# lbroseus/TALC

Measured on AMD Instinct MI355X. Metric: corrected long-read bases/sec (whole node); k-mer-probe HBM GB/s, higher is better.
Workload: dtype u8

## Files before the change

talc_amd/csrc/talc_capi_correct.inc:

```

static uint32_t next_launch_stamp() {
  static std::atomic<uint32_t> launches{0};
  return 0x01000000u + (launches.fetch_add(1) & 0xFFFFFFu);
}
static void ensure_edge_boxes(talc_ctx* c, Stage& st) {
  const uint64_t gap = (uint64_t)c->p.max_border_length + 256;
  const uint32_t seqCap = (uint32_t)align_up((uint64_t)(2.2 * (double)gap) + 4ull * c->p.k + 64, 16);
  const uint64_t need = (uint64_t)st.n_slots * edge_box_bytes(seqCap) + (uint64_t)st.n_slots * 4;
  if (c->sw.edgeTasks == 0 || c->p.max_start_anchors < 2 || c->p.max_start_anchors > EDGE_BOX_ANCHORS ||
      seqCap > (1u << 16) || need > (1ull << 30)) {
    st.boxes.reset(); st.boxes_bytes = 0;
    return;
  }
  if (need > st.boxes_bytes || seqCap != st.box_seq_cap) {
    st.boxes.reset(); st.boxes_bytes = 0;
    if (st.boxes.alloc(need) != hipSuccess) { (void)hipGetLastError(); return; }
    st.boxes_bytes = need; st.box_seq_cap = seqCap;
  }
}

static int ensure_stage(talc_ctx* c, Stage& st, uint32_t maxLen, uint32_t scale, uint32_t n_work) {
  const SearchCaps caps = make_caps(maxLen, c->p.k, scale, scale == 1 ? c->sw.seqArena : 0, scale == 1 && c->sw.tinyCaps);
  hipDeviceProp_t prop;
  HIPCHK(hipGetDeviceProperties(&prop, c->device));
// ... 114 lines not shown
  HIPCHK(hipEventRecord(c->ev[3], s));
  return TALC_OK;
}

static int order_queue(talc_ctx* c, talc_batch* b) {
  if (!b->n_reads) return TALC_OK;
  hipStream_t s = c->stream;
  uint32_t* const hist = c->d_hist.get();
  HIPCHK(hipMemsetAsync(hist, 0, kOrderBuckets * sizeof(uint32_t), s));
  const unsigned nb = (b->n_reads + 255) / 256;
  hipLaunchKernelGGL(k_order_scale, dim3(1), dim3(64), 0, s, batch_stats(c));
  hipLaunchKernelGGL(k_order_hist, dim3(nb), dim3(256), 0, s, b->d_state.get(), b->n_reads, hist, batch_stats(c));
  hipLaunchKernelGGL(k_order_scan, dim3(1), dim3(kOrderBuckets), 0, s, hist);
  hipLaunchKernelGGL(k_order_scatter, dim3(nb), dim3(256), 0, s, b->d_state.get(), b->n_reads, hist, b->d_order.get(), batch_stats(c));
  HIPCHK(hipGetLastError());
  return TALC_OK;
}

static int launch_search(talc_ctx* c, talc_batch* b, const Stage& st, const uint32_t* d_work, uint32_t n_work, const TraceBuf& tb,
                         uint32_t traceRead, bool edgeTasks) {
  hipStream_t s = c->stream;
  HIPCHK(hipMemsetAsync(c->d_queue.get(), 0, kQueueWords * sizeof(uint32_t), s));
  EdgeTaskArgs ea = {};
  ea.test = c->sw.edgeLane ? 0u : kTestNoEdgeLane;
  if (edgeTasks && st.boxes) {
    ea.boxes = st.boxes.get();
    ea.avail = (uint32_t*)(st.boxes.get() + (uint64_t)st.n_slots * edge_box_bytes(st.box_seq_cap));
    ea.seqCap = st.box_seq_cap;
    ea.minWeak = c->sw.edgeTaskMin; ea.heavy = c->sw.edgeTaskHeavy; ea.heavyRounds = c->sw.edgeTaskRounds;
    ea.lingerMod = c->sw.edgeLingerMod; ea.test |= c->sw.edgeRedo ? kTestEdgeRedo : 0u;
    ea.autoSwitch = c->sw.edgeTasks > 0 ? nullptr : batch_stats(c) + kStatBranching;
    HIPCHK(hipMemsetAsync(ea.avail, 0, (uint64_t)st.n_slots * 4, s));
  }
  hipLaunchKernelGGL(k_search, dim3(st.n_slots), dim3(64), 0, s, c->dp, c->view, st.caps, b->d_codes.get(), b->d_offsets.get(),
                     b->d_koff.get(), b->d_cov.get(), b->d_covw.get(), b->d_state.get(), b->d_regions.get(), b->d_regoff.get(), b->d_headcov.get(),
                     c->map ? b->d_regions.get() : nullptr, c->map ? b->d_mapedge.get() : nullptr, b->d_out.get(), b->d_outoff.get(), d_work,
                     n_work, c->d_queue.get(), st.scratch.get(), c->d_counters.get(), tb, traceRead, next_launch_stamp(), ea);
  HIPCHK(hipGetLastError());
  return TALC_OK;
}

static int search_first_pass(talc_ctx* c, talc_batch* b, const TraceBuf& tb, uint32_t traceRead) {
  hipStream_t s = c->stream;
  int rc;
  HIPCHK(hipMemsetAsync(c->d_counters.get(), 0, kCounterWords * sizeof(uint64_t), s));
  HIPCHK(hipMemsetAsync(c->d_counters.get() + kCntFirstStart, 0xFF, sizeof(uint64_t), s));
  HIPCHK(hipMemsetAsync(c->d_counters.get() + kCntQueueDry, 0xFF, sizeof(uint64_t), s));
// ... 483 lines not shown
```

talc_amd/csrc/talc_kernels_search.h:

```cpp
#pragma once
#include "talc_common.h"
#include "talc_kernels_probe.h"
#include "talc_pure.h"
#include "talc_wave.h"

namespace talc {

#define TCAP 288
#define NBUF (2 * TCAP)
#ifndef LDS_DP_CAP
#define LDS_DP_CAP 320
#endif
#ifndef HOT
#define HOT 8
#endif
#ifndef AIMS_LDS
#define AIMS_LDS 16
#endif

enum : uint32_t {
  OVF_ANCHORS = 1, OVF_FULLPATHS = 2, OVF_FULLPOOL = 4, OVF_TRAILS = 8, OVF_SEQ = 16, OVF_OUT = 32, OVF_WEAKPOOL = 64,
  OVF_REGIONS = 128, OVF_DP = 256
};

// ... 10 lines not shown
  uint32_t pfHead, pfTail, pfGapSum, pfFork, pfSolid, pfTicks;
  uint32_t pfGapSq, pfGapMax, pfShortReg, pfSteps;
  uint32_t pfBridges, pfBridgeMax;
  uint32_t pfEdgeTicks, pfAnchors, pfAnchorMax, pfStart;
#endif
};

__host__ __device__ inline uint64_t out_capacity_for(uint64_t L) { return 4 * L + 1024; }

struct FullMeta { uint32_t off, len; int32_t lanc, ranc; double dist; };

static const uint32_t kQueueWords = 768, kQueueFinished = 256, kQueueOpen = 512;

static const uint32_t kOrderBuckets = 1024, kBatchStatsOff = kOrderBuckets, kBatchStatsWords = 256, kHistWords = kBatchStatsOff + kBatchStatsWords;
static const uint32_t kStatGapScale = 128, kStatBranching = 129;

static const uint32_t kCntSteps = 0, kCntCells = 1, kCntProf0 = 2, kCntQueueDry = 124, kCntBusy = 125, kCntFirstStart = 126, kCntLastEnd = 127;
static const uint32_t kCntWaveLog = 128, kCntMaxWaves = 8192, kCounterWords = kCntWaveLog + 2 * kCntMaxWaves;

enum { PF_PROBE = 0, PF_CHILD, PF_AIMS, PF_CYCLE, PF_FFWD, PF_SCOREBR, PF_GARDEN, PF_EVALFULL, PF_XDROP, PF_EXTNW,
       PF_EDGEMISC, PF_ANCHORS, PF_ASSEMBLE, PF_STEPB, PF_STEPE, PF_SRCHB, PF_SRCHE, PF_PROLOG, PF_INITTR, PF_TOTAL, PF_NCALLS, PF_NSTEPS,
       PF_FFLOAD, PF_FFREC, PF_FFFLUSH, PF_FFENTRY, PF_NRECS, PF_RD0, PF_RD1, PF_RD2, PF_RD3, PF_RD4, PF_RD5, PF_RDMAX,
       PF_XSTAGE, PF_XLEV, PF_XSEL, PF_REFB, PF_RESULT, PF_CYQ, PF_CYX, PF_CYHIT, PF_CYFILL,
       PF_SB11, PF_SB12, PF_SB21, PF_SB10, PF_SBOTHER, PF_SEGEN, PF_XCALLS, PF_XNLEV, PF_FSFORK, PF_FSDEAD, PF_FSFILT, PF_FSLIM, PF_FK1, PF_FK2, PF_FKBAIL, PF_FORK, PF_ANCCALLS, PF_ANCITER, PF_TPUB, PF_TOWN, PF_TSTOLEN, PF_TWAIT, PF_TRUN, PF_EA0, PF_EA1, PF_EA2, PF_EA3, PF_EA4, PF_EASUM3, PF_EASUM4, PF_RANCH, PF_RANCHMAX, PF_RBR, PF_RBRMAX, PF_EDGELANE, PF_N };
#define TALC_PF_NAMES {"probe", "child", "aims", "cycle", "ffwd", "scorebr", "garden", "evalfull", "xdrop", "extnw", "edgemisc", \
                       "anchors", "assemble", "stepb*", "stepe*", "srchb*", "srche*", "prolog", "inittr", "total", "#ffcalls", "#ffsteps", \
                       "ff.load", "ff.record", "ff.flush", "ff.entry", "#ffrecords", "#reads<0.25ms", "#reads<1ms", "#reads<4ms", \
                       "#reads<16ms", "#reads<64ms", "#reads>=64ms", "maxread(10ns)", "x.stage", "x.levels", "x.select", "b.ref", "b.result", \
                       "#cyc.query", "#cyc.exact", "#cyc.found", "cyc.fill%sum", \
                       "#stepb 1->1", "#stepb 1->2", "#stepb 2->1", "#stepb 1->0", "#stepb other", "#stepe generic", "#xdrop calls", "#xdrop levels", \
                       "#ffstop fork", "#ffstop deadend", "#ffstop filter", "#ffstop limit/other", "#forkstep 1 child", "#forkstep fork+deadend", "#forkstep bailed", "forkstep", "#anchor lists", "#anchor level tests", \
                       "#edges published", "#anchors by owner", "#anchors by others", "t.owner waits", "t.run by others", \
                       "#edge anchors<1ms", "#edge anchors<4ms", "#edge anchors<16ms", "#edge anchors<64ms", "#edge anchors>=64ms", "ticks anchors 16-64ms", "ticks anchors>=64ms", "(per read) anchors", "(per read) longest anchor", "(per read) bridge attempts", "(per read) longest bridge attempt", "edgelane*"}
static_assert(kCntProf0 + PF_N <= kCntQueueDry, "the profile categories run into the utilisation counters");

struct SearchLimits {
  uint32_t seqCap;
  uint32_t seqArena;
  uint32_t refCap;
  uint32_t edgeCap;
  uint32_t anchCap;
  uint32_t fullCap;
  uint32_t fullPool;
  uint32_t dpCap;
  uint32_t regCap;
  uint32_t weakPool;
};
struct SearchCaps : SearchLimits {
  uint64_t slotBytes;
  uint64_t o_setA, o_setB, o_seqPool, o_ref, o_ancL, o_ancR, o_ancPos, o_fullMeta, o_fullPoolB, o_edgeLong,
      o_edgeShort, o_edgeTmp, o_dp, o_gard, o_regS, o_regE, o_wOff, o_wLen, o_weak, o_wideBloom, o_rowPool, o_regH, o_trace;
};

#ifndef ROW_ARENA_INTS
#define ROW_ARENA_INTS (448 * 1024)
#endif
// ... 466 lines not shown
  s.kmer = (uint64_t*)(meta + TrailSetLayout::kmer); s.nmask = (uint64_t*)(meta + TrailSetLayout::nmask);
  s.dist = (double*)(meta + TrailSetLayout::dist); s.cnt = (uint32_t*)(meta + TrailSetLayout::cnt);
  s.score = (int32_t*)(meta + TrailSetLayout::score); s.fail = (uint32_t*)(meta + TrailSetLayout::fail);
  s.lanc = (int32_t*)(meta + TrailSetLayout::lanc); s.ranc = (int32_t*)(meta + TrailSetLayout::ranc);
  s.buf = (uint32_t*)(meta + TrailSetLayout::buf);
  return s;
}

struct TrailRec { uint64_t kmer, nmask; double dist; uint32_t cnt; int32_t score; uint32_t fail; int32_t lanc, ranc; uint32_t buf; };

#define LSYNC() do { __builtin_amdgcn_fence(__ATOMIC_ACQ_REL, "wavefront"); __builtin_amdgcn_wave_barrier(); } while (0)

__shared__ TrailRec g_hot[2 * HOT];
__shared__ uint64_t g_aimK[AIMS_LDS], g_aimN[AIMS_LDS];
__shared__ uint32_t g_aimPos[AIMS_LDS];
#define BLOOM_WORDS 128
__shared__ unsigned long long g_bloom[BLOOM_WORDS];
__shared__ __attribute__((aligned(16))) int g_dp[3 * LDS_DP_CAP];

struct EdgeCand {
  bool have; double score; double dist; double idscore; uint32_t len; uint32_t lanc, ranc;
};

enum : uint32_t { kTestEdgeRedo = 1u, kTestNoEdgeLane = 2u };

struct Wv {
  DevParams P; TableView T; SearchLimits C;
  const uint8_t* read; uint32_t L, n; const uint2* cov; double lambda;
  TrailSet G[2];
  int ia;
  uint8_t* seqPool;
  uint32_t nBuf;
  unsigned long long freeMask[NBUF / 64];
  uint8_t *ref, *fullPool, *edgeLong, *edgeShort, *edgeTmp, *weak;
  AnchorRec *ancL, *ancR; uint32_t* ancPos;
  FullMeta* fullMeta;
  int *dpG;
  double* gScores; double* gDists; ValIdx* gVal; Rank4* gRank; uint32_t* gKept;
  uint32_t *regS, *regE, *wOff, *wLen;
  int location, dirRight;
  uint32_t Ls, Le, Rs, Re;
  uint32_t weakLen;
  bool complexRegion;
  bool ffPopped;
  int nAncL, nAncR;
  uint32_t refLen;
  int nFull; uint32_t fullUsed;
  EdgeCand best2[2];
  int nEdges;
  unsigned long long cells, steps;
  uint32_t overflow;
  const TraceBuf* tracep;
  bool tracing, traceSteps;
  unsigned long long* wideBloom;
  int* rowPool;
  uint32_t searchNo;
  uint32_t rowStride, rowAvail;
  uint32_t wideMask;
  uint32_t launchStamp;
  const CovWord* covw;
  uint32_t* regH;
  uint32_t LH, RH;
  const uint32_t* headCov;
  uint8_t* refBuf;
  uint8_t* boxes; uint32_t* avail; uint32_t* qwords;
  uint32_t* mapRegions; uint32_t* mapEdge;
  uint32_t boxBytes, boxSeqCap, nSlots, mySlot, nWork, taskMinWeak;
// ... 1630 lines not shown

  flush();
  g_bloom[l] = ((unsigned long long)(uint32_t)bwHi << 32) | (uint32_t)bwLo;
  g_bloom[l + 64] = ((unsigned long long)(uint32_t)bxHi << 32) | (uint32_t)bxLo;
  stepCounter_ = sc0 + (uint32_t)done;
  PROF_COUNT(PF_NCALLS, 1); PROF_COUNT(PF_NSTEPS, done);
  if (done) {
    X.steps += (unsigned long long)done;
    if (l == 0) {
      TrailRec r = r0;
      r.kmer = kmer; r.cnt = cnt; r.dist = dist;
      tr_put(X.ia, 0, r);
    }
  }
  LSYNC();
  return done;
}

template <int P>
TALC_D uint32_t dpp_row_shr(uint32_t v, uint32_t old) {
  return (uint32_t)__builtin_amdgcn_update_dpp((int)old, (int)v, 0x110 + P, 0xF, 0xF, false);
}

struct WalkLanes { uint32_t laneOff, laneShift, laneSingle; int lj; };
struct WalkTip { uint64_t kmer, key; uint32_t hh, cnt; uint32_t ePre; bool havePre; int done, flushed; };
template <bool dirRight, bool WIDEF, class Also>
TALC_D int walk_record(const WalkLanes& WL, WalkTip& W, int room, const uint32_t TALC_AS1* wtab, uint64_t cap, uint32_t K, gu8 seq, int len0,
                       uint32_t* recN, int nAims, uint32_t wideMask, unsigned long long* wideBloom, int& nOK, int& aimIdx, Also also) {
  PROF_DECL;
  const int l = lane_id();
  const uint64_t kmask = (1ULL << (2 * K)) - 1, m1 = (1ULL << (2 * (K - 1))) - 1;
  const uint32_t laneOff = WL.laneOff, laneShift = WL.laneShift, laneSingle = WL.laneSingle;
  const int lj = WL.lj;
  uint64_t& kmer = W.kmer; uint64_t& key = W.key; uint32_t& hh = W.hh; uint32_t& cnt = W.cnt; uint32_t& ePre = W.ePre; bool& havePre = W.havePre;
  int& done = W.done; const int flushed = W.flushed;
  nOK = 0; aimIdx = -1;
    PROF_BEGIN();
    uint64_t slot = ((uint64_t)hh * (uint64_t)(uint32_t)cap) >> 32;
    uint32_t e = havePre ? ePre : wtab[slot * 8 + laneOff];
    havePre = false;
    bool found = true;
    while (true) {
      const uint64_t bk = ((uint64_t)(uint32_t)lane_get((int)e, TALC_WALK_LEVELS + 1) << 32) | (uint32_t)lane_get((int)e, TALC_WALK_LEVELS);
      if (bk == key) break;
      if (bk == kEmptyKey) { found = false; break; }
      if (++slot == cap) slot = 0;
      e = wtab[slot * 8 + laneOff];
    }
    PROF_END(PF_FFLOAD);
    PROF_COUNT(PF_NRECS, 1);
    if (!found) return 0;
    PROF_BEGIN();
    const uint32_t lev = (e >> laneShift) & 0xFFFFu, top = lev & kWalkTopNone;
#ifdef TALC_PROF
    {
      const unsigned long long pm = ballot64((l < TALC_WALK_LEVELS) && (lev & kWalkSingle) != 0u);
      const int j0 = __builtin_ctzll(~pm);
      if (j0 < TALC_WALK_LEVELS && j0 < room) {
        const uint32_t t0 = (uint32_t)lane_get((int)top, j0);
        if (l == 0) g_prof[(t0 >= X.P.MIN_COUNT) ? PF_FSFORK : PF_FSDEAD] += 1;
      }
    }
#endif
    const unsigned long long passMask = ballot64((lev & laneSingle) != 0u);
    nOK = min(__builtin_ctzll(~passMask), room);
    if (nOK == 0) return 0;
    const uint32_t which = (l < TALC_WALK_LEVELS) ? (lev >> kWalkBaseShift) : 0u;
    uint32_t pre = which << (dirRight ? 2 * (TALC_WALK_LEVELS - 1 - lj) : 2 * lj);
    pre |= dpp_row_shr<1>(pre, 0u);
    pre |= dpp_row_shr<2>(pre, 0u);
    pre |= dpp_row_shr<4>(pre, 0u);
    pre |= dpp_row_shr<8>(pre, 0u);
    uint64_t km;
    if (dirRight) km = ((kmer << (2 * (lj + 1))) | (uint64_t)(pre >> (2 * (TALC_WALK_LEVELS - 1 - lj)))) & kmask;
    else km = ((uint64_t)pre << (2 * (K - 1 - (uint32_t)lj))) | (kmer >> (2 * (lj + 1)));
    const uint64_t key2 = dirRight ? (km & m1) : (km >> 2);
    const uint32_t hv = (uint32_t)(table_hash(key2) >> 32);
    {
      const uint64_t slotN = ((uint64_t)(uint32_t)lane_get((int)hv, TALC_WALK_LEVELS - 1) * (uint64_t)(uint32_t)cap) >> 32;
      ePre = wtab[slotN * 8 + laneOff];
    }
    bool dup = dpp_row_shr<1>(hv, ~hv) == hv;
    dup |= dpp_row_shr<2>(hv, ~hv) == hv;
    dup |= dpp_row_shr<3>(hv, ~hv) == hv;
    dup |= dpp_row_shr<4>(hv, ~hv) == hv;
    dup |= dpp_row_shr<5>(hv, ~hv) == hv;
    dup |= dpp_row_shr<6>(hv, ~hv) == hv;
    dup |= dpp_row_shr<7>(hv, ~hv) == hv;
    dup |= dpp_row_shr<8>(hv, ~hv) == hv;
    dup |= dpp_row_shr<9>(hv, ~hv) == hv;
    dup |= dpp_row_shr<10>(hv, ~hv) == hv;
    dup |= dpp_row_shr<11>(hv, ~hv) == hv;
    static_assert(TALC_WALK_LEVELS == 12, "the lane roles above are written for 12 levels (+ 2 key lanes) in a 16-lane row");
    const int bwi = (int)(hv >> 25);
    const unsigned long long bm = (1ull << ((hv >> 19) & 63u)) | (1ull << ((hv >> 13) & 63u));
    bool seen = (g_bloom[bwi] & bm) == bm;
    unsigned long long* const wideW = WIDEF ? wideBloom + wide_word(hv, wideMask) : nullptr;
    const unsigned long long bmW = WIDEF ? wide_bits(hv) : 0ull;
    if (WIDEF) {
      const bool ask = seen && (l < TALC_WALK_LEVELS);
      if (ballot64(ask) != 0ull) { const unsigned long long bvW = ask ? wide_load(wideW) : 0ull; seen = ask && ((bvW & bmW) == bmW); }
    }
    const unsigned long long hitMask = ballot64(seen || dup) | (1ull << TALC_WALK_LEVELS);
    const int hitLevel = __builtin_ctzll(hitMask);
    aimIdx = -1;
    if (nAims > 0 && nAims <= AIMS_LDS && hitLevel < nOK) {
      const uint64_t kmH = ((uint64_t)(uint32_t)lane_get((int)(uint32_t)(km >> 32), hitLevel) << 32) | (uint32_t)lane_get((int)(uint32_t)km, hitLevel);
      const unsigned long long am = ballot64((l < nAims) && (g_aimK[l < AIMS_LDS ? l : 0] == kmH) && (g_aimN[l < AIMS_LDS ? l : 0] == 0ull));
      if (am != 0ull) aimIdx = (int)__builtin_ctzll(am);
    }
    if (hitLevel < nOK && aimIdx < 0) PROF_COUNT(PF_FSFILT, 1);
    nOK = min(nOK, hitLevel);
    const int nTake = nOK + (aimIdx >= 0 ? 1 : 0);
    if (nTake == 0) return 0;
    if (l < nTake) {
      atomicOr(&g_bloom[bwi], bm);
      if (WIDEF) wide_or(wideW, bmW);
      recN[done - flushed + l] = top;
      seq[len0 + done + l] = (uint8_t)which;
      also(len0 + done + l, which);
    }
    const int last = nTake - 1;
    kmer = ((uint64_t)(uint32_t)lane_get((int)(uint32_t)(km >> 32), last) << 32) | (uint32_t)lane_get((int)(uint32_t)km, last);
    key = dirRight ? (kmer & m1) : (kmer >> 2);
    hh = (uint32_t)lane_get((int)hv, last);
    havePre = (last == TALC_WALK_LEVELS - 1);
    cnt = (uint32_t)lane_get((int)top, last);
    done += nTake;
    LSYNC();
    PROF_END(PF_FFREC);
  return nTake;
}
TALC_D void walk_flush(WalkTip& W, uint32_t* recN, uint32_t& cFlush, double& dist) {
  const int l = lane_id();
  int& done = W.done; int& flushed = W.flushed;
  const int n = done - flushed;
  if (n <= 0) return;
  PROF_DECL; PROF_BEGIN();
  const uint32_t cn = (l < n) ? recN[l] : 1u;
  const uint32_t cprev = (l == 0) ? cFlush : ((l < n) ? recN[l - 1] : 1u);
  const double term = fabs((double)cprev - (double)cn) / sqrt((double)cprev);
  double* recT = (double*)(g_dp + 64);
  recT[l] = term;
  LSYNC();
#pragma unroll 8
  for (int j = 0; j < n; ++j) dist = dist + recT[j];
  cFlush = (uint32_t)lane_get((int)cn, n - 1);
  flushed = done;
  LSYNC();
  PROF_END(PF_FFFLUSH);
}

template <bool dirRight, bool WIDEF>
TALC_D int fast_forward_walk(int len_, uint32_t& stepCounter_, uint32_t PATH_MAXLENGTH_, bool edge_) {
  PROF_DECL2;
  PROF_BEGIN2();
  const DevParams& P = X.P;
  const int l = lane_id();
  const bool edge = uni((int)edge_) != 0;
  if (uni((int)(X.traceSteps)) != 0) return 0;
  const TrailRec r0 = tr_get(X.ia, 0);
  if (uni64(r0.nmask) != 0ull) return 0;
  const uint32_t K = (uint32_t)uni((int)P.K), CHECK = (uint32_t)uni((int)P.CHECK_INTERVAL);
  const uint32_t seqCap = (uint32_t)uni((int)X.C.seqCap), PMAX = (uint32_t)uni((int)PATH_MAXLENGTH_);
  const uint64_t cap = uni64(X.T.capacity);
  const uint32_t TALC_AS1* wtab = (const uint32_t TALC_AS1*)uni_ptr(dirRight ? X.T.walkRight : X.T.walkLeft);
  const uint32_t wideMask = WIDEF ? (uint32_t)uni((int)X.wideMask) : 0u;
  unsigned long long* const wideBloom = WIDEF ? (unsigned long long*)uni_ptr(X.wideBloom) : nullptr;
  const uint64_t m1 = (1ULL << (2 * (K - 1))) - 1;
  WalkTip W;
  uint64_t& kmer = W.kmer; uint32_t& cnt = W.cnt;
  kmer = uni64(r0.kmer);
  cnt = (uint32_t)uni((int)r0.cnt);
// ... 9 lines not shown
  int lanc = uni((int)r0.lanc), ranc = uni((int)r0.ranc);
  bool popped = false;
  uint32_t* recN = (uint32_t*)g_dp;
  uint32_t cFlush = cnt;
  double dist = r0.dist;
  int& done = W.done; int& flushed = W.flushed;
  done = 0; flushed = 0;

  auto flush = [&]() { walk_flush(W, recN, cFlush, dist); };

  WalkLanes WL;
  WL.laneOff = (l < TALC_WALK_LEVELS) ? (uint32_t)(2 + (l >> 1)) : (l == TALC_WALK_LEVELS + 1 ? 1u : 0u);
  WL.laneShift = (l < TALC_WALK_LEVELS && (l & 1)) ? 16u : 0u;
  WL.lj = min(l, TALC_WALK_LEVELS - 1);
  WL.laneSingle = (l < TALC_WALK_LEVELS) ? kWalkSingle : 0u;
  W.key = dirRight ? (kmer & m1) : (kmer >> 2);
  W.hh = (uint32_t)(table_hash(W.key) >> 32);
  PROF_END2(PF_FFENTRY);
  W.ePre = 0;
  W.havePre = false;
  while (done < maxSteps) {
    if (done - flushed > 64 - TALC_WALK_LEVELS) flush();
    int nOK, aimIdx;
    const int nTake = walk_record<dirRight, WIDEF>(WL, W, maxSteps - done, wtab, cap, K, seq, len0, recN, nAims, wideMask, wideBloom, nOK, aimIdx,
                                                   [](int, uint32_t) {});
    if (nTake == 0) break;
    if (aimIdx >= 0) {
      flush();
      WSYNC();
      const int apos = (int)g_aimPos[aimIdx];
      if (dirRight) ranc = apos; else lanc = apos;
      const uint32_t clen = (uint32_t)(len0 + done);
      if (X.nFull >= (int)X.C.fullCap) X.overflow |= OVF_FULLPATHS;
      else if (X.fullUsed + clen > X.C.fullPool) X.overflow |= OVF_FULLPOOL;
      else {
        wave_copy_bytes(X.fullPool + X.fullUsed, (const uint8_t*)seq, clen, false);
        if (l == 0) X.fullMeta[X.nFull] = FullMeta{X.fullUsed, clen, lanc, ranc, dist / ((double)clen + 0.01)};
        X.fullUsed += (clen + 15u) & ~15u;
        X.nFull++;
        WSYNC();
      }
      if (X.overflow) break;
      if (clen > X.refLen) { popped = true; break; }
      continue;
    }
    if (nOK < TALC_WALK_LEVELS) break;
  }
  flush();
  stepCounter_ = sc0 + (uint32_t)done;
  PROF_COUNT(PF_NCALLS, 1); PROF_COUNT(PF_NSTEPS, done);
  if (done) {
    X.steps += (unsigned long long)done;
    if (l == 0) {
      TrailRec r = r0;
      r.kmer = kmer; r.cnt = cnt; r.dist = dist; r.lanc = lanc; r.ranc = ranc;
      tr_put(X.ia, 0, r);
    }
  }
  if (popped) { pool_free((int)r0.buf); X.ffPopped = true; }
  LSYNC();
  return done;
}

TALC_DN int fast_forward_steps(int len, uint32_t& stepCounter, uint32_t PATH_MAXLENGTH, bool edge) {
  return uni((int)X.dirRight) ? fast_forward_dir<true>(len, stepCounter, PATH_MAXLENGTH, edge)
                              : fast_forward_dir<false>(len, stepCounter, PATH_MAXLENGTH, edge);
}
TALC_DNC int fast_forward_wide(int len, uint32_t& stepCounter, uint32_t PATH_MAXLENGTH, bool edge) {
  return uni((int)X.dirRight) ? fast_forward_walk<true, true>(len, stepCounter, PATH_MAXLENGTH, edge)
                              : fast_forward_walk<false, true>(len, stepCounter, PATH_MAXLENGTH, edge);
}
TALC_DN int fast_forward(int len, uint32_t& stepCounter, uint32_t PATH_MAXLENGTH, bool edge) {
  if (uni((int)(X.T.walkRight != nullptr && X.P.MIN_COUNT < kWalkTopNone)) != 0)
  {
    if (uni((int)X.wideMask) != 0) [[clang::musttail]] return fast_forward_wide(len, stepCounter, PATH_MAXLENGTH, edge);
    return uni((int)X.dirRight) ? fast_forward_walk<true, false>(len, stepCounter, PATH_MAXLENGTH, edge)
                                : fast_forward_walk<false, false>(len, stepCounter, PATH_MAXLENGTH, edge);
  }
  [[clang::musttail]] return fast_forward_steps(len, stepCounter, PATH_MAXLENGTH, edge);
}

struct EdgeLaneRet { int len; uint32_t stepCounter; int xdrop; int ff; int dead; int leafFell; };
constexpr int kLaneStageOff = 768;

template <bool dirRight>
TALC_D EdgeLaneRet edge_lane_dir(int len_, uint32_t stepCounter_, uint32_t PATH_MAXLENGTH_, int xdrop_) {
  PROF_DECL;
  const DevParams& P = X.P;
  const int l = lane_id();
  EdgeLaneRet R;
  R.len = uni(len_); R.stepCounter = (uint32_t)uni((int)stepCounter_); R.xdrop = uni(xdrop_); R.ff = 0; R.dead = 0; R.leafFell = 0;
  if (uni((int)(X.traceSteps)) != 0) return R;
  const TrailRec r0 = tr_get(X.ia, 0);
  if (uni64(r0.nmask) != 0ull) return R;
  const uint32_t K = (uint32_t)uni((int)P.K), CHECK = (uint32_t)uni((int)P.CHECK_INTERVAL);
  const uint32_t seqCap = (uint32_t)uni((int)X.C.seqCap), PMAX = (uint32_t)uni((int)PATH_MAXLENGTH_);
  const uint32_t MAXFAIL = (uint32_t)uni((int)P.MAX_BORDER_FAILURES);
  const uint64_t cap = uni64(X.T.capacity);
// ... 33 lines not shown
  WalkLanes WL;
  WL.laneOff = (l < TALC_WALK_LEVELS) ? (uint32_t)(2 + (l >> 1)) : (l == TALC_WALK_LEVELS + 1 ? 1u : 0u);
  WL.laneShift = (l < TALC_WALK_LEVELS && (l & 1)) ? 16u : 0u;
  WL.lj = min(l, TALC_WALK_LEVELS - 1);
  WL.laneSingle = (l < TALC_WALK_LEVELS) ? kWalkSingle : 0u;
  W.key = dirRight ? (kmer & m1) : (kmer >> 2);
  W.hh = (uint32_t)(table_hash(W.key) >> 32);
  W.ePre = 0;
  W.havePre = false;
  uint32_t phase = sc0 % CHECK;

  while (true) {
    const uint32_t sc = sc0 + (uint32_t)done;
    const int roundStart = done;
    int lim = done;
    if (sc < PMAX && (uint32_t)(len0 + done) < seqCap)
      lim = done + (int)min(min(PMAX - sc, seqCap - (uint32_t)(len0 + done)), CHECK - phase);
#ifdef TALC_PROF
    ++rounds;
#endif
    while (done < lim) {
      if (done - flushed > 64 - TALC_WALK_LEVELS) flush();
      int nOK, aimIdx;
      const int nTake = walk_record<dirRight, false>(WL, W, lim - done, wtab, cap, K, seq, len0, recN, 0, 0u, nullptr, nOK, aimIdx,
                                                     [&](int pos, uint32_t base) { const int qi = pos - S; if (stageFits && qi < dlen) stage[qi] = (uint8_t)base; });
      if (nTake == 0) break;
      if (nOK < TALC_WALK_LEVELS) break;
    }
    R.ff = done - roundStart;
    phase += (uint32_t)R.ff;
    if (phase == CHECK) phase = 0;
    if (R.ff == 0 || phase != 0) break;
    const int len = len0 + done, x = xdrop + 2;
    const int qlen = len - S;
    if (!stageFits || len > refLen) break;
    if (min(max(x, 0), qlen) + min(max(x, 0), dlen) + 1 > 63) break;
    PROF_BEGIN();
    PROF_COUNT(PF_XCALLS, 1);
    if (!staged) {
      WSYNC();
      stage_copy(stage, (gcu8)seq + S, qlen);
      stage_copy(stage + qpad, (gcu8)uni_ptr(X.ref) + S, dlen);
      if (l == 0) stage[qpad + dlen] = 0xF1;
      staged = true;
    }
    if (l == 0) stage[qlen] = 0xF0;
    int extCols = 0, extRows = 0, extScore = 0;
// ... 17 lines not shown
  }

  flush();
  R.len = len0 + done; R.stepCounter = sc0 + (uint32_t)done; R.xdrop = xdrop;
  PROF_COUNT(PF_NCALLS, rounds); PROF_COUNT(PF_NSTEPS, done);
  X.cells += ncells;
  if (done) {
    X.steps += (unsigned long long)done;
    if (l == 0) {
      TrailRec r;
      r.kmer = kmer; r.nmask = 0ull; r.dist = dist; r.cnt = cnt; r.score = score; r.fail = fail; r.lanc = lanc; r.ranc = ranc; r.buf = buf;
      tr_put(X.ia, 0, r);
    }
  }
  if (R.dead | R.leafFell) WSYNC();
  else LSYNC();
  return R;
}
TALC_DN EdgeLaneRet edge_lane(int len, uint32_t stepCounter, uint32_t PATH_MAXLENGTH, int xdrop) {
  return uni((int)X.dirRight) ? edge_lane_dir<true>(len, stepCounter, PATH_MAXLENGTH, xdrop)
                              : edge_lane_dir<false>(len, stepCounter, PATH_MAXLENGTH, xdrop);
}

TALC_DN int fork_step(int len_, uint32_t sc_, uint32_t PMAX_) {
  PROF_DECL;
  PROF_BEGIN();
  const DevParams& P = X.P;
  const int l = lane_id();
  const int len = uni(len_);
  const uint32_t sc = (uint32_t)uni((int)sc_), PMAX = (uint32_t)uni((int)PMAX_);
  if (uni((int)X.traceSteps) != 0) return 0;
  if ((uint32_t)uni((int)P.MAXB) < 2u || (uint32_t)uni((int)P.MAX_INNER_PATHS) < 2u) return 0;
  const TrailRec r0 = tr_get(X.ia, 0);
  if (uni64(r0.nmask) != 0ull) return 0;
  const uint32_t K = (uint32_t)uni((int)P.K), MINC = (uint32_t)uni((int)P.MIN_COUNT), seqCap = (uint32_t)uni((int)X.C.seqCap);
  if (!(sc < PMAX) || (uint32_t)len + 1u > seqCap) return 0;
  const bool dirRight = uni(X.dirRight) != 0;
  const uint64_t kmask = (1ULL << (2 * K)) - 1, m1 = (1ULL << (2 * (K - 1))) - 1;
  const uint64_t kmer = uni64(r0.kmer);
  const uint32_t cnt = (uint32_t)uni((int)r0.cnt);
  auto child_of = [&](uint64_t km, uint32_t b) -> uint64_t {
    return dirRight ? (((km << 2) | (uint64_t)b) & kmask) : (((uint64_t)b << (2 * (K - 1))) | (km >> 2));
  };
  auto get64 = [&](uint64_t v, int src) -> uint64_t {
    return ((uint64_t)(uint32_t)lane_get((int)(uint32_t)(v >> 32), src) << 32) | (uint32_t)lane_get((int)(uint32_t)v, src);
  };
  bool tipInTable;
  const ModelThresholds mtTip = model_thresholds(cnt, tipInTable);
  if (uni((int)tipInTable) == 0) return 0;
  const uint64_t kmMine = (l == 4) ? kmer : child_of(kmer, (uint32_t)(l & 3));
  const uint64_t keyMine = dirRight ? (kmMine & m1) : (kmMine >> 2);
  const Bucket* tab = dirRight ? X.T.right : X.T.left;
  const uint64_t cap = X.T.capacity;
// ... 496 lines not shown
  X.best2[0] = best0; X.best2[1] = best1;
  if (uni(win0) >= 0) edge_box_take(box, uni(win0), 0, best0.len);
  if (uni(win1) >= 0) edge_box_take(box, uni(win1), 1, best1.len);
  WSYNC();
}

TALC_D bool queue_is_dry() {
  uint32_t v = 0;
  if (lane_id() == 0) v = aload32(X.qwords);
  return (uint32_t)uni((int)v) >= X.nWork;
}

TALC_D int edge_ctx_load(uint8_t* box) {
  const int l = lane_id();
  const uint32_t* box32 = (const uint32_t*)box;
  LSYNC();
  if (l < 24) g_dp[l] = (int)aload32(box32 + l);
  LSYNC();
  const EdgeBoxHdr* h = (const EdgeBoxHdr*)g_dp;
  const int limit = uni((int)h->limit);
  X.read = h->read; X.cov = h->cov; X.covw = h->covw; X.lambda = h->lambda; X.L = h->L; X.n = h->n;
  X.location = (int)h->location; X.dirRight = (int)h->dirRight;
  X.Ls = h->Ls; X.Le = h->Le; X.Rs = h->Rs; X.Re = h->Re; X.LH = h->LH; X.RH = h->RH; X.weakLen = h->weakLen;
  X.ffPopped = false; X.tracing = false; X.traceSteps = false;
  X.nAncL = X.dirRight ? limit : 0; X.nAncR = X.dirRight ? 0 : limit;
  LSYNC();
  return limit;
}

TALC_DNC bool edge_task_steal(int tries);

TALC_DNC int edge_anchors_as_tasks(const AnchorRec* anchors_, int s0_, int limit_) {
  const AnchorRec* anchors = uni_ptr(anchors_);
  const int s0 = uni(s0_), limit = uni(limit_);
  const int l = lane_id();
  const uint32_t me = (uint32_t)uni((int)X.mySlot);
  uint8_t* box = uni_ptr(edge_box(me));
  uint32_t* box32 = (uint32_t*)box;
  uint32_t* done = box32 + offsetof(EdgeBoxHdr, done) / 4;
  const int first = s0 > 0 ? s0 - 1 : s0;
  if (s0 > 0) {
    const uint32_t cap = (uint32_t)uni((int)X.boxSeqCap);
    if ((X.best2[0].have && X.best2[0].len > cap) || (X.best2[1].have && X.best2[1].len > cap)) return 0;
    edge_box_store(box, s0 - 1, 0u);
  }
  LSYNC();
  {
// ... 652 lines not shown
```

talc_amd/csrc/talc_switches.h:

```cpp
#pragma once
#include <algorithm>
#include <cstdint>
#include <cstdlib>
#include <string>

namespace talc {

struct Switches {
  int timing = 0;
  bool hostParse = false;
  int walk = -1;
  uint32_t filterBits = 20;
  uint32_t tableSlotsX10 = 0;
  uint32_t searchSlots = 0;
  uint32_t seqArena = 0;
  bool tinyCaps = false;
  bool failRetryAlloc = false;
  int edgeTasks = -1;
  uint32_t edgeTaskMin = 150, edgeTaskHeavy = 200, edgeTaskRounds = 0xFFFF, edgeLingerMod = 16;
  bool edgeRedo = false;
  bool edgeLane = true;
  bool traceSteps = false;
  uint32_t fakeGpus = 0;
  std::string profReads;
  bool profPrint = false, profSlow = false;
};

inline Switches read_switches() {
  auto given = [](const char* name) { return std::getenv(name) != nullptr; };
  auto num = [](const char* name, long unset) { const char* e = std::getenv(name); return e ? std::atol(e) : unset; };
  auto clamped = [&](const char* name, long unset, long lo, long hi) { return (uint32_t)std::min(std::max(num(name, unset), lo), hi); };
  Switches s;
  if (const char* e = std::getenv("TALC_TIMING")) s.timing = e[0] == '2' ? 2 : 1;
  s.hostParse = given("TALC_HOST_PARSE");
  if (given("TALC_WALK")) s.walk = num("TALC_WALK", 0) != 0 ? 1 : 0;
  if (const char* e = std::getenv("TALC_FILTER_BITS")) s.filterBits = (uint32_t)std::min<uint64_t>(64, std::max<uint64_t>(4, std::strtoull(e, nullptr, 10)));
  if (const char* e = std::getenv("TALC_TABLE_SLOTS_X10")) { const uint64_t v = std::strtoull(e, nullptr, 10); if (v >= 20 && v <= 80) s.tableSlotsX10 = (uint32_t)v; }
  s.searchSlots = clamped("TALC_SEARCH_SLOTS", 0, 0, 1L << 30);
  s.seqArena = clamped("TALC_SEQ_ARENA", 0, 0, 1L << 30);
  s.tinyCaps = num("TALC_TEST_TINY_CAPS", 0) > 0;
  s.failRetryAlloc = given("TALC_TEST_FAIL_RETRY_ALLOC");
  if (given("TALC_EDGE_TASKS")) { const long v = num("TALC_EDGE_TASKS", 0); s.edgeTasks = v == 0 ? 0 : v > 0 ? 1 : -1; }
  s.edgeTaskMin = clamped("TALC_EDGE_TASK_MIN", 150, 0, 1L << 30);
  s.edgeTaskHeavy = clamped("TALC_EDGE_TASK_HEAVY", 200, 0, 1L << 30);
  s.edgeTaskRounds = clamped("TALC_EDGE_TASK_ROUNDS", 0xFFFF, 0, 0xFFFF);
  s.edgeLingerMod = clamped("TALC_EDGE_LINGER_MOD", 16, 1, 1L << 20);
  s.edgeRedo = given("TALC_TEST_EDGE_REDO");
  s.edgeLane = num("TALC_TEST_EDGE_LANE", 1) != 0;
  s.traceSteps = num("TALC_TRACE_STEPS", 0) != 0;
  s.fakeGpus = clamped("TALC_FAKE_GPUS", 0, 0, 1L << 20);
  if (const char* e = std::getenv("TALC_PROF_READS")) s.profReads = e;
  s.profPrint = given("TALC_PROF_PRINT");
  s.profSlow = given("TALC_PROF_SLOW");
  return s;
}

}
```

Before: 4.793 billion.

## Add bridge lane walk that continues past Bloom-filter hits via cycle check

```diff
diff --git a/talc_amd/csrc/talc_capi_correct.inc b/talc_amd/csrc/talc_capi_correct.inc
--- a/talc_amd/csrc/talc_capi_correct.inc
+++ b/talc_amd/csrc/talc_capi_correct.inc
@@ -160,7 +160,7 @@
   hipStream_t s = c->stream;
   HIPCHK(hipMemsetAsync(c->d_queue.get(), 0, kQueueWords * sizeof(uint32_t), s));
   EdgeTaskArgs ea = {};
-  ea.test = c->sw.edgeLane ? 0u : kTestNoEdgeLane;
+  ea.test = (c->sw.edgeLane ? 0u : kTestNoEdgeLane) | (c->sw.bridgeLane ? 0u : kTestNoBridgeLane);
   if (edgeTasks && st.boxes) {
     ea.boxes = st.boxes.get();
     ea.avail = (uint32_t*)(st.boxes.get() + (uint64_t)st.n_slots * edge_box_bytes(st.box_seq_cap));
diff --git a/talc_amd/csrc/talc_kernels_search.h b/talc_amd/csrc/talc_kernels_search.h
--- a/talc_amd/csrc/talc_kernels_search.h
+++ b/talc_amd/csrc/talc_kernels_search.h
@@ -56,7 +56,7 @@
        PF_EDGEMISC, PF_ANCHORS, PF_ASSEMBLE, PF_STEPB, PF_STEPE, PF_SRCHB, PF_SRCHE, PF_PROLOG, PF_INITTR, PF_TOTAL, PF_NCALLS, PF_NSTEPS,
        PF_FFLOAD, PF_FFREC, PF_FFFLUSH, PF_FFENTRY, PF_NRECS, PF_RD0, PF_RD1, PF_RD2, PF_RD3, PF_RD4, PF_RD5, PF_RDMAX,
        PF_XSTAGE, PF_XLEV, PF_XSEL, PF_REFB, PF_RESULT, PF_CYQ, PF_CYX, PF_CYHIT, PF_CYFILL,
-       PF_SB11, PF_SB12, PF_SB21, PF_SB10, PF_SBOTHER, PF_SEGEN, PF_XCALLS, PF_XNLEV, PF_FSFORK, PF_FSDEAD, PF_FSFILT, PF_FSLIM, PF_FK1, PF_FK2, PF_FKBAIL, PF_FORK, PF_ANCCALLS, PF_ANCITER, PF_TPUB, PF_TOWN, PF_TSTOLEN, PF_TWAIT, PF_TRUN, PF_EA0, PF_EA1, PF_EA2, PF_EA3, PF_EA4, PF_EASUM3, PF_EASUM4, PF_RANCH, PF_RANCHMAX, PF_RBR, PF_RBRMAX, PF_EDGELANE, PF_N };
+       PF_SB11, PF_SB12, PF_SB21, PF_SB10, PF_SBOTHER, PF_SEGEN, PF_XCALLS, PF_XNLEV, PF_FSFORK, PF_FSDEAD, PF_FSFILT, PF_FSLIM, PF_FK1, PF_FK2, PF_FKBAIL, PF_FORK, PF_ANCCALLS, PF_ANCITER, PF_TPUB, PF_TOWN, PF_TSTOLEN, PF_TWAIT, PF_TRUN, PF_EA0, PF_EA1, PF_EA2, PF_EA3, PF_EA4, PF_EASUM3, PF_EASUM4, PF_RANCH, PF_RANCHMAX, PF_RBR, PF_RBRMAX, PF_EDGELANE, PF_BRIDGELANE, PF_LNFILT, PF_LNCYC, PF_N };
 #define TALC_PF_NAMES {"probe", "child", "aims", "cycle", "ffwd", "scorebr", "garden", "evalfull", "xdrop", "extnw", "edgemisc", \
                        "anchors", "assemble", "stepb*", "stepe*", "srchb*", "srche*", "prolog", "inittr", "total", "#ffcalls", "#ffsteps", \
                        "ff.load", "ff.record", "ff.flush", "ff.entry", "#ffrecords", "#reads<0.25ms", "#reads<1ms", "#reads<4ms", \
@@ -65,7 +65,8 @@
                        "#stepb 1->1", "#stepb 1->2", "#stepb 2->1", "#stepb 1->0", "#stepb other", "#stepe generic", "#xdrop calls", "#xdrop levels", \
                        "#ffstop fork", "#ffstop deadend", "#ffstop filter", "#ffstop limit/other", "#forkstep 1 child", "#forkstep fork+deadend", "#forkstep bailed", "forkstep", "#anchor lists", "#anchor level tests", \
                        "#edges published", "#anchors by owner", "#anchors by others", "t.owner waits", "t.run by others", \
-                       "#edge anchors<1ms", "#edge anchors<4ms", "#edge anchors<16ms", "#edge anchors<64ms", "#edge anchors>=64ms", "ticks anchors 16-64ms", "ticks anchors>=64ms", "(per read) anchors", "(per read) longest anchor", "(per read) bridge attempts", "(per read) longest bridge attempt", "edgelane*"}
+                       "#edge anchors<1ms", "#edge anchors<4ms", "#edge anchors<16ms", "#edge anchors<64ms", "#edge anchors>=64ms", "ticks anchors 16-64ms", "ticks anchors>=64ms", "(per read) anchors", "(per read) longest anchor", "(per read) bridge attempts", "(per read) longest bridge attempt", "edgelane*", \
+                       "bridgelane*", "#lane filter checks", "#lane cycles found"}
 static_assert(kCntProf0 + PF_N <= kCntQueueDry, "the profile categories run into the utilisation counters");
 
 struct SearchLimits {
@@ -578,7 +579,7 @@
   bool have; double score; double dist; double idscore; uint32_t len; uint32_t lanc, ranc;
 };
 
-enum : uint32_t { kTestEdgeRedo = 1u, kTestNoEdgeLane = 2u };
+enum : uint32_t { kTestEdgeRedo = 1u, kTestNoEdgeLane = 2u, kTestNoBridgeLane = 4u };
 
 struct Wv {
   DevParams P; TableView T; SearchLimits C;
@@ -599,6 +600,7 @@
   uint32_t weakLen;
   bool complexRegion;
   bool ffPopped;
+  uint8_t laneStop;
   int nAncL, nAncR;
   uint32_t refLen;
   int nFull; uint32_t fullUsed;
@@ -2275,11 +2277,14 @@
   return (uint32_t)__builtin_amdgcn_update_dpp((int)old, (int)v, 0x110 + P, 0xF, 0xF, false);
 }
 
+enum : int { kWalkNoRecord = 1, kWalkNotSingle = 2, kWalkFilterHit = 3 };
+struct WalkStop { int why; uint32_t base, top, hv; uint64_t km;
+                  bool resumed; };
 struct WalkLanes { uint32_t laneOff, laneShift, laneSingle; int lj; };
 struct WalkTip { uint64_t kmer, key; uint32_t hh, cnt; uint32_t ePre; bool havePre; int done, flushed; };
 template <bool dirRight, bool WIDEF, class Also>
 TALC_D int walk_record(const WalkLanes& WL, WalkTip& W, int room, const uint32_t TALC_AS1* wtab, uint64_t cap, uint32_t K, gu8 seq, int len0,
-                       uint32_t* recN, int nAims, uint32_t wideMask, unsigned long long* wideBloom, int& nOK, int& aimIdx, Also also) {
+                       uint32_t* recN, int nAims, uint32_t wideMask, unsigned long long* wideBloom, int& nOK, int& aimIdx, WalkStop& S, Also also) {
   PROF_DECL;
   const int l = lane_id();
   const uint64_t kmask = (1ULL << (2 * K)) - 1, m1 = (1ULL << (2 * (K - 1))) - 1;
@@ -2302,14 +2307,14 @@
     }
     PROF_END(PF_FFLOAD);
     PROF_COUNT(PF_NRECS, 1);
-    if (!found) return 0;
+    if (!found) { S.why = kWalkNoRecord; return 0; }
     PROF_BEGIN();
     const uint32_t lev = (e >> laneShift) & 0xFFFFu, top = lev & kWalkTopNone;
 #ifdef TALC_PROF
     {
       const unsigned long long pm = ballot64((l < TALC_WALK_LEVELS) && (lev & kWalkSingle) != 0u);
       const int j0 = __builtin_ctzll(~pm);
-      if (j0 < TALC_WALK_LEVELS && j0 < room) {
+      if (j0 < TALC_WALK_LEVELS && j0 < room && !S.resumed) {
         const uint32_t t0 = (uint32_t)lane_get((int)top, j0);
         if (l == 0) g_prof[(t0 >= X.P.MIN_COUNT) ? PF_FSFORK : PF_FSDEAD] += 1;
       }
@@ -2317,7 +2322,7 @@
 #endif
     const unsigned long long passMask = ballot64((lev & laneSingle) != 0u);
     nOK = min(__builtin_ctzll(~passMask), room);
-    if (nOK == 0) return 0;
+    if (nOK == 0) { S.why = kWalkNotSingle; return 0; }
     const uint32_t which = (l < TALC_WALK_LEVELS) ? (lev >> kWalkBaseShift) : 0u;
     uint32_t pre = which << (dirRight ? 2 * (TALC_WALK_LEVELS - 1 - lj) : 2 * lj);
     pre |= dpp_row_shr<1>(pre, 0u);
@@ -2362,10 +2367,15 @@
       const unsigned long long am = ballot64((l < nAims) && (g_aimK[l < AIMS_LDS ? l : 0] == kmH) && (g_aimN[l < AIMS_LDS ? l : 0] == 0ull));
       if (am != 0ull) aimIdx = (int)__builtin_ctzll(am);
     }
-    if (hitLevel < nOK && aimIdx < 0) PROF_COUNT(PF_FSFILT, 1);
+    if (hitLevel < nOK && aimIdx < 0 && !S.resumed) PROF_COUNT(PF_FSFILT, 1);
     nOK = min(nOK, hitLevel);
     const int nTake = nOK + (aimIdx >= 0 ? 1 : 0);
-    if (nTake == 0) return 0;
+    if (nTake == 0) {
+      S.why = kWalkFilterHit;
+      S.base = (uint32_t)lane_get((int)which, 0); S.top = (uint32_t)lane_get((int)top, 0); S.hv = (uint32_t)lane_get((int)hv, 0);
+      S.km = ((uint64_t)(uint32_t)lane_get((int)(uint32_t)(km >> 32), 0) << 32) | (uint32_t)lane_get((int)(uint32_t)km, 0);
+      return 0;
+    }
     if (l < nTake) {
       atomicOr(&g_bloom[bwi], bm);
       if (WIDEF) wide_or(wideW, bmW);
@@ -2402,6 +2412,30 @@
   flushed = done;
   LSYNC();
   PROF_END(PF_FFFLUSH);
+}
+
+template <bool dirRight>
+TALC_D bool walk_bridge_at_aim(int aimIdx, gu8 seq, uint32_t clen, int& lanc, int& ranc, double dist, bool& popped) {
+  const int l = lane_id();
+  WSYNC();
+  const int apos = (int)g_aimPos[aimIdx];
+  if (dirRight) ranc = apos; else lanc = apos;
+  if (X.nFull >= (int)X.C.fullCap) X.overflow |= OVF_FULLPATHS;
+  else if (X.fullUsed + clen > X.C.fullPool) X.overflow |= OVF_FULLPOOL;
+  else {
+    {
+      gu8 dst = (gu8)uni_ptr(X.fullPool + X.fullUsed);
+#pragma unroll 2
+      for (uint32_t i = (uint32_t)l; i < clen; i += 64) dst[i] = seq[i];
+    }
+    if (l == 0) X.fullMeta[X.nFull] = FullMeta{X.fullUsed, clen, lanc, ranc, dist / ((double)clen + 0.01)};
+    X.fullUsed += (clen + 15u) & ~15u;
+    X.nFull++;
+    WSYNC();
+  }
+  if (X.overflow) return false;
+  if (clen > X.refLen) { popped = true; return false; }
+  return true;
 }
 
 template <bool dirRight, bool WIDEF>
@@ -2457,26 +2491,13 @@
   while (done < maxSteps) {
     if (done - flushed > 64 - TALC_WALK_LEVELS) flush();
     int nOK, aimIdx;
-    const int nTake = walk_record<dirRight, WIDEF>(WL, W, maxSteps - done, wtab, cap, K, seq, len0, recN, nAims, wideMask, wideBloom, nOK, aimIdx,
+    WalkStop S; S.resumed = false;
+    const int nTake = walk_record<dirRight, WIDEF>(WL, W, maxSteps - done, wtab, cap, K, seq, len0, recN, nAims, wideMask, wideBloom, nOK, aimIdx, S,
                                                    [](int, uint32_t) {});
     if (nTake == 0) break;
     if (aimIdx >= 0) {
       flush();
-      WSYNC();
-      const int apos = (int)g_aimPos[aimIdx];
-      if (dirRight) ranc = apos; else lanc = apos;
-      const uint32_t clen = (uint32_t)(len0 + done);
-      if (X.nFull >= (int)X.C.fullCap) X.overflow |= OVF_FULLPATHS;
-      else if (X.fullUsed + clen > X.C.fullPool) X.overflow |= OVF_FULLPOOL;
-      else {
-        wave_copy_bytes(X.fullPool + X.fullUsed, (const uint8_t*)seq, clen, false);
-        if (l == 0) X.fullMeta[X.nFull] = FullMeta{X.fullUsed, clen, lanc, ranc, dist / ((double)clen + 0.01)};
-        X.fullUsed += (clen + 15u) & ~15u;
-        X.nFull++;
-        WSYNC();
-      }
-      if (X.overflow) break;
-      if (clen > X.refLen) { popped = true; break; }
+      if (!walk_bridge_at_aim<dirRight>(aimIdx, seq, (uint32_t)(len0 + done), lanc, ranc, dist, popped)) break;
       continue;
     }
     if (nOK < TALC_WALK_LEVELS) break;
@@ -2505,10 +2526,12 @@
   return uni((int)X.dirRight) ? fast_forward_walk<true, true>(len, stepCounter, PATH_MAXLENGTH, edge)
                               : fast_forward_walk<false, true>(len, stepCounter, PATH_MAXLENGTH, edge);
 }
+TALC_DN int bridge_lane(int len, uint32_t& stepCounter, uint32_t PATH_MAXLENGTH, bool);
 TALC_DN int fast_forward(int len, uint32_t& stepCounter, uint32_t PATH_MAXLENGTH, bool edge) {
   if (uni((int)(X.T.walkRight != nullptr && X.P.MIN_COUNT < kWalkTopNone)) != 0)
   {
     if (uni((int)X.wideMask) != 0) [[clang::musttail]] return fast_forward_wide(len, stepCounter, PATH_MAXLENGTH, edge);
+    if (uni((int)(!edge && (X.taskTest & kTestNoBridgeLane) == 0u)) != 0) [[clang::musttail]] return bridge_lane(len, stepCounter, PATH_MAXLENGTH, edge);
     return uni((int)X.dirRight) ? fast_forward_walk<true, false>(len, stepCounter, PATH_MAXLENGTH, edge)
                                 : fast_forward_walk<false, false>(len, stepCounter, PATH_MAXLENGTH, edge);
   }
@@ -2588,7 +2611,8 @@
     while (done < lim) {
       if (done - flushed > 64 - TALC_WALK_LEVELS) flush();
       int nOK, aimIdx;
-      const int nTake = walk_record<dirRight, false>(WL, W, lim - done, wtab, cap, K, seq, len0, recN, 0, 0u, nullptr, nOK, aimIdx,
+      WalkStop WS; WS.resumed = false;
+      const int nTake = walk_record<dirRight, false>(WL, W, lim - done, wtab, cap, K, seq, len0, recN, 0, 0u, nullptr, nOK, aimIdx, WS,
                                                      [&](int pos, uint32_t base) { const int qi = pos - S; if (stageFits && qi < dlen) stage[qi] = (uint8_t)base; });
       if (nTake == 0) break;
       if (nOK < TALC_WALK_LEVELS) break;
@@ -2652,6 +2676,130 @@
                               : edge_lane_dir<false>(len, stepCounter, PATH_MAXLENGTH, xdrop);
 }
 
+enum : int { kLaneStopOther = 0,
+             kLaneStopNotSingle = 1,
+             kLaneStopFilter = 2,
+             kLaneStopCycle = 3 };
+
+template <bool dirRight>
+TALC_D int bridge_lane_dir(int len_, uint32_t& stepCounter_, uint32_t PATH_MAXLENGTH_) {
+  PROF_DECL2;
+  PROF_BEGIN2();
+  const DevParams& P = X.P;
+  const int l = lane_id();
+  int why = kLaneStopOther;
+  if (uni((int)(X.traceSteps)) != 0) return 0;
+  const TrailRec r0 = tr_get(X.ia, 0);
+  if (uni64(r0.nmask) != 0ull) return 0;
+  const uint32_t K = (uint32_t)uni((int)P.K);
+  const uint32_t seqCap = (uint32_t)uni((int)X.C.seqCap), PMAX = (uint32_t)uni((int)PATH_MAXLENGTH_);
+  const uint64_t cap = uni64(X.T.capacity);
+  const uint32_t TALC_AS1* wtab = (const uint32_t TALC_AS1*)uni_ptr(dirRight ? X.T.walkRight : X.T.walkLeft);
+  const uint64_t m1 = (1ULL << (2 * (K - 1))) - 1;
+  WalkTip W;
+  uint64_t& kmer = W.kmer; uint32_t& cnt = W.cnt;
+  kmer = uni64(r0.kmer);
+  cnt = (uint32_t)uni((int)r0.cnt);
+  const int len0 = uni(len_);
+  const uint32_t sc0 = (uint32_t)uni((int)stepCounter_);
+  int maxSteps = 0;
+  if (sc0 < PMAX && (uint32_t)len0 < seqCap) maxSteps = (int)min(PMAX - sc0, seqCap - (uint32_t)len0);
+  const uint32_t buf = (uint32_t)uni((int)r0.buf);
+  gu8 seq = (gu8)uni_ptr(X.seqPool + (uint64_t)buf * X.C.seqCap);
+  const int nAims = uni(dirRight ? X.nAncR : X.nAncL);
+  const bool mayCheck = nAims <= AIMS_LDS && (uint32_t)uni((int)P.MAXB) >= 1u;
+  int lanc = uni((int)r0.lanc), ranc = uni((int)r0.ranc);
+  const int score = uni((int)r0.score);
+  const uint32_t fail = (uint32_t)uni((int)r0.fail);
+  bool popped = false;
+  uint32_t* recN = (uint32_t*)g_dp;
+  uint32_t cFlush = cnt;
+  double dist = r0.dist;
+  int& done = W.done; int& flushed = W.flushed;
+  done = 0; flushed = 0;
+
+  auto flush = [&]() { walk_flush(W, recN, cFlush, dist); };
+
+  WalkLanes WL;
+  WL.laneOff = (l < TALC_WALK_LEVELS) ? (uint32_t)(2 + (l >> 1)) : (l == TALC_WALK_LEVELS + 1 ? 1u : 0u);
+  WL.laneShift = (l < TALC_WALK_LEVELS && (l & 1)) ? 16u : 0u;
+  WL.lj = min(l, TALC_WALK_LEVELS - 1);
+  WL.laneSingle = (l < TALC_WALK_LEVELS) ? kWalkSingle : 0u;
+  W.key = dirRight ? (kmer & m1) : (kmer >> 2);
+  W.hh = (uint32_t)(table_hash(W.key) >> 32);
+  W.ePre = 0;
+  W.havePre = false;
+  WalkStop S; S.why = 0; S.resumed = false;
+  PROF_END2(PF_FFENTRY);
+
+  while (done < maxSteps) {
+    if (done - flushed > 64 - TALC_WALK_LEVELS) flush();
+    int nOK, aimIdx;
+    const int nTake = walk_record<dirRight, false>(WL, W, maxSteps - done, wtab, cap, K, seq, len0, recN, nAims, 0u, nullptr, nOK, aimIdx, S,
+                                                   [](int, uint32_t) {});
+    if (nTake != 0) {
+      if (aimIdx >= 0) {
+        flush();
+        if (!walk_bridge_at_aim<dirRight>(aimIdx, seq, (uint32_t)(len0 + done), lanc, ranc, dist, popped)) break;
+      }
+#ifdef TALC_PROF
+      S.resumed = aimIdx < 0 && nOK < TALC_WALK_LEVELS;
+#endif
+      continue;
+    }
+    if (S.why != kWalkFilterHit) { why = (S.why == kWalkNotSingle) ? kLaneStopNotSingle : kLaneStopOther; break; }
+    why = kLaneStopFilter;
+    if (!mayCheck) break;
+    PROF_COUNT(PF_LNFILT, 1);
+    const int len = len0 + done;
+    if (l == 0) seq[len] = (uint8_t)S.base;
+    if (len > (int)K) {
+      WSYNC();
+      const uint8_t* const parent = (const uint8_t*)seq;
+      const uint8_t* const pat = parent + (len + 1 - (int)K);
+      bool cyc;
+      if (dirRight) cyc = wave_find_window(parent, len, pat, (int)K, false) > 0;
+      else { const int q = wave_find_window(parent, len, pat, (int)K, true); cyc = q >= 0 && q != len - (int)K; }
+      if (uni((int)cyc) != 0) { PROF_COUNT(PF_LNCYC, 1); why = kLaneStopCycle; break; }
+    }
+    if (l == 0) recN[done - flushed] = S.top;
+    kmer = S.km;
+    W.key = dirRight ? (kmer & m1) : (kmer >> 2);
+    W.hh = S.hv;
+    cnt = S.top;
+    done += 1;
+    LSYNC();
+    why = kLaneStopOther;
+#ifdef TALC_PROF
+    S.resumed = false;
+#endif
+  }
+
+  flush();
+  stepCounter_ = sc0 + (uint32_t)done;
+  PROF_COUNT(PF_NCALLS, 1); PROF_COUNT(PF_NSTEPS, done);
+  if (l == 0) X.laneStop = (why == kLaneStopFilter || why == kLaneStopCycle) ? (uint8_t)1 : (uint8_t)0;
+  if (done) {
+    X.steps += (unsigned long long)done;
+    if (l == 0) {
+      TrailRec r;
+      r.kmer = kmer; r.nmask = 0ull; r.dist = dist; r.cnt = cnt; r.score = score; r.fail = fail; r.lanc = lanc; r.ranc = ranc; r.buf = buf;
+      tr_put(X.ia, 0, r);
+    }
+  }
+  if (popped) { pool_free((int)buf); X.ffPopped = true; }
+  LSYNC();
+  return done;
+}
+TALC_DN int bridge_lane(int len, uint32_t& stepCounter, uint32_t PATH_MAXLENGTH, bool) {
+  PROF_DECL2;
+  PROF_BEGIN2();
+  const int done = uni((int)X.dirRight) ? bridge_lane_dir<true>(len, stepCounter, PATH_MAXLENGTH)
+                                        : bridge_lane_dir<false>(len, stepCounter, PATH_MAXLENGTH);
+  PROF_END2(PF_BRIDGELANE);
+  return done;
+}
+
 TALC_DN int fork_step(int len_, uint32_t sc_, uint32_t PMAX_) {
   PROF_DECL;
   PROF_BEGIN();
@@ -2659,6 +2807,11 @@
   const int l = lane_id();
   const int len = uni(len_);
   const uint32_t sc = (uint32_t)uni((int)sc_), PMAX = (uint32_t)uni((int)PMAX_);
+  if (uni((int)X.laneStop) != 0) {
+    if (l == 0) X.laneStop = 0;
+    LSYNC();
+    return 0;
+  }
   if (uni((int)X.traceSteps) != 0) return 0;
   if ((uint32_t)uni((int)P.MAXB) < 2u || (uint32_t)uni((int)P.MAX_INNER_PATHS) < 2u) return 0;
   const TrailRec r0 = tr_get(X.ia, 0);
@@ -3201,7 +3354,7 @@
   X.read = h->read; X.cov = h->cov; X.covw = h->covw; X.lambda = h->lambda; X.L = h->L; X.n = h->n;
   X.location = (int)h->location; X.dirRight = (int)h->dirRight;
   X.Ls = h->Ls; X.Le = h->Le; X.Rs = h->Rs; X.Re = h->Re; X.LH = h->LH; X.RH = h->RH; X.weakLen = h->weakLen;
-  X.ffPopped = false; X.tracing = false; X.traceSteps = false;
+  X.ffPopped = false; X.laneStop = 0; X.tracing = false; X.traceSteps = false;
   X.nAncL = X.dirRight ? limit : 0; X.nAncR = X.dirRight ? 0 : limit;
   LSYNC();
   return limit;
diff --git a/talc_amd/csrc/talc_switches.h b/talc_amd/csrc/talc_switches.h
--- a/talc_amd/csrc/talc_switches.h
+++ b/talc_amd/csrc/talc_switches.h
@@ -20,6 +20,7 @@
   uint32_t edgeTaskMin = 150, edgeTaskHeavy = 200, edgeTaskRounds = 0xFFFF, edgeLingerMod = 16;
   bool edgeRedo = false;
   bool edgeLane = true;
+  bool bridgeLane = true;
   bool traceSteps = false;
   uint32_t fakeGpus = 0;
   std::string profReads;
@@ -47,6 +48,7 @@
   s.edgeLingerMod = clamped("TALC_EDGE_LINGER_MOD", 16, 1, 1L << 20);
   s.edgeRedo = given("TALC_TEST_EDGE_REDO");
   s.edgeLane = num("TALC_TEST_EDGE_LANE", 1) != 0;
+  s.bridgeLane = num("TALC_TEST_BRIDGE_LANE", 1) != 0;
   s.traceSteps = num("TALC_TRACE_STEPS", 0) != 0;
   s.fakeGpus = clamped("TALC_FAKE_GPUS", 0, 0, 1L << 20);
   if (const char* e = std::getenv("TALC_PROF_READS")) s.profReads = e;
```

After: 4.662 billion. 0.973x the previous value.
